# FuxiComputerVision/Nefii

Hardware: AMD Instinct MI355X
Metric: training rays/sec (Step-2 material opt) (higher is better)
Workload: dtype f16x3; 1 GPU; cfg3; parallelism=dp1, trace_tier=True, bracket_staged_eval=False, split_fp8=False, step_graph=False, cycle_batches=4, trace_prefetch=3, nonfinite_steps=0

## Files before the change

nefii_amd/csrc/nefii_mlp.hip:

```cpp
#include "mlp_tile.h"

using namespace nefii;

#define HIP_CHECK_LAUNCH()                       \
    do {                                         \
        hipError_t _e = hipGetLastError();       \
        if (_e != hipSuccess) return (int)_e;    \
    } while (0)

static inline int round32(int v) { return (v + 31) & ~31; }
static inline int pad_hidden(int v) { return v <= 32 ? round32(v) : (v + 63) & ~63; }
extern "C" int nefii_padded_width(int v) { return v < 0 ? NEFII_E_ARG : pad_hidden(v); }

extern "C" int nefii_abi_version(void) { return NEFII_ABI_VERSION; }

struct PackGeom {
    int n_out, k_in, kx, ke, n_pad, x_src0, x_len, e_src0, e_len;
    float scale;
    __device__ __forceinline__ int src_col(int kk) const {
        if (kk < kx) return kk < x_len ? x_src0 + kk : -1;
        const int e = kk - kx;
        return e < e_len ? e_src0 + e : -1;
    }
    __device__ __forceinline__ float at(const float *__restrict__ W, int n, int kk) const {
// ... 771 lines not shown
                        const int j = ft * QT + qt;
                        float4v hv;
#pragma unroll
                        for (int k = 0; k < 4; ++k) {
                            const float z = __builtin_fmaf(acc[j][k], inv_scale, bs[k]);
                            hv[k] = ACT == NEFII_ACT_ELU ? elu_fast(z) : act_fwd(z, ACT);
                        }
                        const int64_t row = base + 16 * qt + (lane & 15);
                        if (row < n) {
                            if (stash) *reinterpret_cast<float4v *>(stash + ((size_t)l * n + row) * stash_stride + f0) = hv;
                            if (pre_last) {
#pragma unroll
                                for (int k = 0; k < 4; ++k)
                                    if (f0 + k < L.n_out) hidden_out[(size_t)row * hid_stride + f0 + k] = hv[k];
                            }
                        }
                        const float4v hs = hv * A16_SCALE;
                        const half4 hi = __builtin_convertvector(hs, half4);
                        phi[j] = hi;
                        plo[j] = __builtin_convertvector(hs - __builtin_convertvector(hi, float4v), half4);
                        if (H16 && stash16 && row < n)
                            *reinterpret_cast<half4 *>(stash16 + ((size_t)l * n + row) * stash_stride + f0) = hi;
                    }
                }
            };
            if (m.act == NEFII_ACT_RELU)
                epilogue(std::integral_constant<int, NEFII_ACT_RELU>{});
            else if (m.act == NEFII_ACT_ELU)
                epilogue(std::integral_constant<int, NEFII_ACT_ELU>{});
            else
                epilogue(std::integral_constant<int, NEFII_ACT_SOFTPLUS100>{});
            __syncthreads();
            _Float16 *xh = lds.Xh + (EP - L.n_pad), *xl = lds.Xl + (EP - L.n_pad);
#pragma unroll
            for (int ft = 0; ft < 4; ++ft) {
                const int f0 = 64 * wave + 16 * ft + 4 * (lane >> 4);
#pragma unroll
                for (int qt = 0; qt < QT; ++qt) {
                    const int query = 16 * qt + (lane & 15);
                    *reinterpret_cast<half4 *>(xh + query * XP + f0) = phi[ft * QT + qt];
                    *reinterpret_cast<half4 *>(xl + query * XP + f0) = plo[ft * QT + qt];
                }
            }
            __syncthreads();
        }
        {
            const int r = lane & 31, h = lane >> 5;
            const nefii_layer &L = m.layer[NH];
            const half8 *wl = reinterpret_cast<const half8 *>(L.w_f16x3) + lane;
            const int ksw = (L.k_x >> 4) / NW;
            f32x16 acc2[RT];
#pragma unroll
            for (int rt = 0; rt < RT; ++rt)
#pragma unroll
                for (int i = 0; i < 16; ++i) acc2[rt][i] = 0.f;
            for (int u = 0; u < ksw; ++u) {
                const int s = wave * ksw + u;
                const half8 wh = wl[(size_t)s * 128], wlo = wl[(size_t)s * 128 + 64];
#pragma unroll
                for (int rt = 0; rt < RT; ++rt) {
                    const int rowc = 32 * rt + r < ROWS ? 32 * rt + r : ROWS - 1;
                    const half8 xh8 = *reinterpret_cast<const half8 *>(lds.Xh + rowc * XP + 8 * h + 16 * s);
                    const half8 xl8 = *reinterpret_cast<const half8 *>(lds.Xl + rowc * XP + 8 * h + 16 * s);
                    acc2[rt] = __builtin_amdgcn_mfma_f32_32x32x16_f16(wh, xh8, acc2[rt], 0, 0, 0);
                    acc2[rt] = __builtin_amdgcn_mfma_f32_32x32x16_f16(wlo, xh8, acc2[rt], 0, 0, 0);
                    acc2[rt] = __builtin_amdgcn_mfma_f32_32x32x16_f16(wh, xl8, acc2[rt], 0, 0, 0);
                }
            }
            __syncthreads();
            float *psum = reinterpret_cast<float *>(lds.Xl);
#pragma unroll
            for (int rt = 0; rt < RT; ++rt)
                if (32 * rt + r < ROWS) {
#pragma unroll
                    for (int i = 0; i < 4; ++i) psum[(wave * ROWS + 32 * rt + r) * 8 + i + 4 * h] = acc2[rt][i];
                }
            __syncthreads();
            for (int i = tid; i < ROWS * 8; i += 512) {
                const int p = i >> 3, c = i & 7;
                if (c < L.n_out && base + p < n) {
                    float sum = 0.f;
#pragma unroll
                    for (int w = 0; w < NW; ++w) sum += psum[(w * ROWS + p) * 8 + c];
                    const float z = sum * inv_scale + L.bias[c];
                    if (stash) stash[((size_t)NH * n + base + p) * stash_stride + c] = z;
                    if (H16 && z_last) z_last[(size_t)(base + p) * 8 + c] = z;
                    out[(size_t)(base + p) * out_stride + c] = head_fwd(z, m.head);
                }
            }
            __syncthreads();
            for (int i = tid; i < NW * ROWS * 8; i += 512) reinterpret_cast<uint32_t *>(lds.Xl)[i] = 0u;
            __syncthreads();
        }
    }
}

static int check_mlp16(const nefii_mlp *m, bool bwd) {
    int rc = check_mlp(m, false);
    if (rc) return rc;
    for (int l = 0; l < m->n_layers; ++l) {
        if (!m->layer[l].w_f16x3) return NEFII_E_ARG;
        if (bwd && l > 0 && !m->layer[l].w_bwd_f16x3) return NEFII_E_ARG;
        if ((m->layer[l].k_x | m->layer[l].k_e | m->layer[l].n_pad) & 15) return NEFII_E_SHAPE;
    }
    return 0;
}

static bool mlp_stream_enabled() {
    static const bool v = env_int("NEFII_MLP_STREAM", 1) != 0;
    return v;
}
static bool mlp_streams_both_ways(const nefii_mlp *m) {
    return m->w_stream && mlp_stream_enabled() && mstream_shape(m) && mstream_units_bwd(m) > 0;
}
static dim3 stream_grid(int64_t n) {
    const int64_t t = (n + 63) / 64;
    return dim3((int)(t < 256 ? t : 256));
}

template <bool H16>
static int launch_forward16q(const nefii_mlp *h_mlp, const float *in_a, const float *in_b, const float *in_c, const float *feat,
                             int64_t n, float *out, int out_stride, float *hidden_out, int hid_stride, void *stash,
                             int stash_stride, float *z_last, void *x0_16, void *stream) {
    const auto kernel = mstream_shape(h_mlp) == 64 ? mlp_forward16q_kernel<4, 64, H16> : mlp_forward16q_kernel<4, 96, H16>;
    hipLaunchKernelGGL(kernel, stream_grid(n), dim3(512), 0, (hipStream_t)stream, *h_mlp, in_a, in_b, in_c, feat, n, out,
                       out_stride, hidden_out, hid_stride, stash, stash_stride, z_last, (_Float16 *)x0_16, mstream_units(h_mlp));
    HIP_CHECK_LAUNCH();
    return 0;
}

extern "C" int nefii_mlp_forward_f16(const nefii_mlp *h_mlp, const float *in_a, const float *in_b, const float *in_c,
                                     const float *feat, int64_t n, float *out, int out_stride, float *hidden_out,
                                     int hid_stride, float *stash, int stash_stride, int single_pass, void *stream) {
    int rc = check_mlp16(h_mlp, false);
    if (rc) return rc;
    if (n <= 0) return 0;
    if (!out) return NEFII_E_ARG;
    const int64_t n_tiles = (n + TILE - 1) / TILE;
    if (!single_pass && h_mlp->w_stream && mlp_stream_enabled() && mstream_shape(h_mlp))
        return launch_forward16q<false>(h_mlp, in_a, in_b, in_c, feat, n, out, out_stride, hidden_out, hid_stride, stash,
                                        stash_stride, nullptr, nullptr, stream);
    if (single_pass)
        hipLaunchKernelGGL(mlp_forward16_kernel<true>, dim3(grid_for(n_tiles, 1)), dim3(WG), 0, (hipStream_t)stream, *h_mlp,
                           in_a, in_b, in_c, feat, n, out, out_stride, hidden_out, hid_stride, stash, stash_stride);
    else
        hipLaunchKernelGGL(mlp_forward16_kernel<false>, dim3(grid_for(n_tiles, 1)), dim3(WG), 0, (hipStream_t)stream, *h_mlp,
                           in_a, in_b, in_c, feat, n, out, out_stride, hidden_out, hid_stride, stash, stash_stride);
    HIP_CHECK_LAUNCH();
    return 0;
}

extern "C" int nefii_mlp_h16_supported(const nefii_mlp *h_mlp) {
    if (!h_mlp || check_mlp16(h_mlp, true)) return 0;
    return mlp_streams_both_ways(h_mlp);
}

extern "C" int nefii_mlp_x0_width(const nefii_mlp *h_mlp) {
    if (!nefii_mlp_h16_supported(h_mlp)) return 0;
    return h_mlp->layer[0].k_x + mstream_shape(h_mlp);
}

extern "C" int nefii_mlp_forward_f16h(const nefii_mlp *h_mlp, const float *in_a, const float *in_b, const float *in_c,
                                      const float *feat, int64_t n, float *out, int out_stride, float *hidden_out,
                                      int hid_stride, void *stash16, int stash_stride, float *z_last, void *x0_16,
                                      void *stream) {
    int rc = check_mlp16(h_mlp, false);
    if (rc) return rc;
    if (!nefii_mlp_h16_supported(h_mlp)) return NEFII_E_SHAPE;
    if (n <= 0) return 0;
    if (!out || !stash16 || !z_last || (stash_stride & 3)) return NEFII_E_ARG;
    return launch_forward16q<true>(h_mlp, in_a, in_b, in_c, feat, n, out, out_stride, hidden_out, hid_stride, stash16,
                                   stash_stride, z_last, x0_16, stream);
}

__global__ void grad_scale_kernel(const float *__restrict__ d, int64_t count, float *__restrict__ scale) {
    __shared__ float wmax[16];
    float mx = 0.f;
    for (int64_t i = threadIdx.x; i < count; i += blockDim.x) {
        const float v = fabsf(d[i]);
        mx = (v < 3.0e38f && v > mx) ? v : mx;
    }
#pragma unroll
    for (int o = 32; o > 0; o >>= 1) mx = fmaxf(mx, __shfl_xor(mx, o));
    if ((threadIdx.x & 63) == 0) wmax[threadIdx.x >> 6] = mx;
    __syncthreads();
    if (threadIdx.x == 0) {
        for (int w = 1; w < (int)(blockDim.x >> 6); ++w) mx = fmaxf(mx, wmax[w]);
        float s = 1.f;
        if (mx > 0.f) {
            int e;
            frexpf(mx, &e);
            e = 8 - e;
            e = e < -40 ? -40 : (e > 60 ? 60 : e);
            s = ldexpf(1.f, e);
        }
        scale[0] = s;
    }
}

__global__ void grad_scale_head_kernel(const float *__restrict__ d, int out_stride, const float *__restrict__ pre, int pre_stride,
                                       int64_t n, int n_out, int head, float *__restrict__ scale) {
    __shared__ float wmax[16];
    float mx = 0.f;
    const int64_t count = n * n_out;
    for (int64_t i = threadIdx.x; i < count; i += blockDim.x) {
        const int64_t p = i / n_out;
        const int c = (int)(i - p * n_out);
        const float dv = d[p * out_stride + c], z = pre[p * pre_stride + c];
        const float v = fabsf(dv);
        const float hv = fabsf(dv * head_bwd_from_out(head_fwd(z, head), z, head)) * 0.125f;
        mx = (v < 3.0e38f && v > mx) ? v : mx;
        mx = (hv < 3.0e38f && hv > mx) ? hv : mx;
    }
#pragma unroll
    for (int o = 32; o > 0; o >>= 1) mx = fmaxf(mx, __shfl_xor(mx, o));
    if ((threadIdx.x & 63) == 0) wmax[threadIdx.x >> 6] = mx;
    __syncthreads();
    if (threadIdx.x == 0) {
        for (int w = 1; w < (int)(blockDim.x >> 6); ++w) mx = fmaxf(mx, wmax[w]);
        float s = 1.f;
        if (mx > 0.f) {
            int e;
            frexpf(mx, &e);
            e = 8 - e;
            e = e < -40 ? -40 : (e > 60 ? 60 : e);
            s = ldexpf(1.f, e);
        }
        scale[0] = s;
    }
}

extern "C" int nefii_mlp_grad_scale_head(const float *d_out, int out_stride, const float *pre, int pre_stride, int64_t n,
                                         int n_out, int head, float *scale, void *stream) {
    if (!d_out || !pre || !scale || n < 0 || n_out < 1 || out_stride < n_out || pre_stride < n_out) return NEFII_E_ARG;
    if (head < NEFII_HEAD_NONE || head > NEFII_HEAD_RELU_INIT) return NEFII_E_ARG;
    hipLaunchKernelGGL(grad_scale_head_kernel, dim3(1), dim3(1024), 0, (hipStream_t)stream, d_out, out_stride, pre, pre_stride, n,
                       n_out, head, scale);
    HIP_CHECK_LAUNCH();
    return 0;
}

extern "C" int nefii_mlp_grad_scale(const float *d_out, int64_t count, float *scale, void *stream) {
    if (!d_out || !scale || count < 0) return NEFII_E_ARG;
    hipLaunchKernelGGL(grad_scale_kernel, dim3(1), dim3(1024), 0, (hipStream_t)stream, d_out, count, scale);
    HIP_CHECK_LAUNCH();
    return 0;
}

__global__ __launch_bounds__(256, 2) void mlp_backward16_kernel(nefii_mlp m, const float *__restrict__ d_out,
                                                                int out_stride, const float *__restrict__ stash,
                                                                int stash_stride, int64_t n, float *__restrict__ dz,
                                                                int dz_stride, const float *__restrict__ scale) {
    __shared__ _Float16 Xh[TILE * XS16];
    const int tid = threadIdx.x;
    const int Lm1 = m.n_layers - 1;
    const float S = scale[0];
    const float inv = 1.f / (W16_SCALE * S);
    const int64_t n_tiles = (n + TILE - 1) / TILE;
    for (int64_t tile = blockIdx.x; tile < n_tiles; tile += gridDim.x) {
        const int64_t base = tile * TILE;
        {
            const nefii_layer &L = m.layer[Lm1];
            for (int i = tid; i < TILE * L.n_pad; i += WG) {
                const int p = i / L.n_pad, c = i - p * L.n_pad;
                float v = 0.f;
                if (base + p < n && c < L.n_out) {
                    const float pre = stash[((size_t)Lm1 * n + base + p) * stash_stride + c];
                    const float y = head_fwd(pre, m.head);
                    v = d_out[(size_t)(base + p) * out_stride + c] * head_bwd_from_out(y, pre, m.head);
                }
                Xh[p * XS16 + c] = (_Float16)(v * S);
                if (base + p < n) dz[((size_t)Lm1 * n + base + p) * dz_stride + c] = v;
            }
        }
        __syncthreads();
        for (int l = Lm1; l >= 1; --l) {
            const nefii_layer &L = m.layer[l];
            f32x16 acc[4];
            const int wave = __builtin_amdgcn_readfirstlane(tid >> 6), lane = tid & 63;
            const int NTs = (L.k_x + L.k_e) >> 5, ntc = L.k_x >> 5;
            int ntw = (ntc - wave + 3) >> 2;
            if (ntw < 0) ntw = 0;
            zero_acc(acc);
            gemm_block16<true>(Xh, Xh, XS16, L.n_pad >> 4, reinterpret_cast<const half8 *>(L.w_bwd_f16x3), NTs, wave, lane,
                               ntw, acc);
            __syncthreads();
            NEFII_ACT_SWITCH(m.act, {
                NEFII_FOR_ACC(acc, ntw, {
                    const bool live = (base + row) < n;
                    float v = 0.f;
                    if (live) {
                        const float hprev = stash[((size_t)(l - 1) * n + base + row) * stash_stride + col];
                        v = val * inv * act_bwd_from_out(hprev, ACT);
                        dz[((size_t)(l - 1) * n + base + row) * dz_stride + col] = v;
                    }
                    Xh[row * XS16 + col] = (_Float16)(v * S);
                })
            })
            __syncthreads();
        }
    }
}

template <bool H16>
__global__ __launch_bounds__(512, 2) void mlp_backward16s_kernel(nefii_mlp m, const float *__restrict__ d_out, int out_stride,
                                                                const void *__restrict__ stash_v, int stash_stride,
                                                                const float *__restrict__ z_last, int64_t n,
                                                                void *__restrict__ dz_v, int dz_stride,
                                                                const float *__restrict__ scale, size_t stream_off, int G) {
    NEFII_CLAIM_SIMD_2();
    const float *const stash = static_cast<const float *>(stash_v);
    const _Float16 *const stash16 = static_cast<const _Float16 *>(stash_v);
    float *const dz = static_cast<float *>(dz_v);
    _Float16 *const dz16 = static_cast<_Float16 *>(dz_v);
    constexpr int QT = 4, FT = 4, ROWS = 64, XP = QGeo<4>::XP, NJ = FT * QT;
    __shared__ LdsS<4, ROWS> lds;
    const int tid = threadIdx.x;
    const int wave = __builtin_amdgcn_readfirstlane(tid >> 6), lane = tid & 63;
    const int Lm1 = m.n_layers - 1;
    const float S = scale[0];
    const float inv = 1.f / (W16_SCALE * S);
    const int64_t n_tiles = (n + ROWS - 1) / ROWS;
    {
        uint32_t *z = reinterpret_cast<uint32_t *>(&lds);
        for (int i = tid; i < (int)(sizeof(lds) / 4); i += 512) z[i] = 0u;
    }
    SStage<4> b[4];
    PCursor cur;
    cur.bytes = (unsigned)G * 4096;
    cur.base = reinterpret_cast<const half8 *>(m.w_stream) + stream_off + (size_t)wave * G * 256 + lane;
    cur.off = 0;
#pragma unroll
    for (int u = 0; u < 3; ++u) sload<4>(b[u], cur);
    const _Float16 *qh0 = lds.Xh + (lane & 15) * XP + 8 * (lane >> 4);
    __syncthreads();
    for (int64_t tile = blockIdx.x; tile < n_tiles; tile += gridDim.x) {
        const int64_t base = tile * ROWS;
        {
            const nefii_layer &L = m.layer[Lm1];
            const int kpad = mb_units(L) * 32;
            for (int i = tid; i < ROWS * kpad; i += 512) {
                const int p = i / kpad, c = i - p * kpad;
                float v = 0.f;
                if (base + p < n && c < L.n_pad) {
                    if (c < L.n_out) {
                        const float pre = H16 ? z_last[(size_t)(base + p) * 8 + c]
                                              : stash[((size_t)Lm1 * n + base + p) * stash_stride + c];
                        const float y = head_fwd(pre, m.head);
                        v = d_out[(size_t)(base + p) * out_stride + c] * head_bwd_from_out(y, pre, m.head);
                    }
                    if (H16) dz16[((size_t)Lm1 * n + base + p) * dz_stride + c] = (_Float16)(v * S);
                    else dz[((size_t)Lm1 * n + base + p) * dz_stride + c] = v;
                }
                lds.Xh[p * XP + c] = (_Float16)(v * S);
            }
        }
        __syncthreads();
        for (int l = Lm1; l >= 1; --l) {
            const nefii_layer &L = m.layer[l];
            const int units = mb_units(L);
            asm volatile("" ::"s"(units));
            __builtin_amdgcn_s_waitcnt(0x0070);
            __builtin_amdgcn_sched_barrier(0);
            f32x4 acc[NJ];
#pragma unroll
            for (int j = 0; j < NJ; ++j)
#pragma unroll
                for (int i = 0; i < 4; ++i) acc[j][i] = 0.f;
            SAct<QT> a[2];
            sload_a<QT, XP>(a[0], qh0, 0);
            sgemm<QT, FT, true>(units, b, a, cur, qh0, acc);
            half4 phi[NJ];
            const float *sp = stash + (size_t)(l - 1) * n * stash_stride;
            float *dp = dz + (size_t)(l - 1) * n * dz_stride;
            const _Float16 *sp16 = stash16 + (size_t)(l - 1) * n * stash_stride;
            _Float16 *dp16 = dz16 + (size_t)(l - 1) * n * dz_stride;
            auto epilogue = [&](auto actc) {
                constexpr int ACT = decltype(actc)::value;
#pragma unroll
                for (int ft = 0; ft < FT; ++ft) {
                    const int f0 = 64 * wave + 16 * ft + 4 * (lane >> 4);
#pragma unroll
                    for (int qt = 0; qt < QT; ++qt) {
                        const int j = ft * QT + qt;
                        const int64_t row = base + 16 * qt + (lane & 15);
                        float4v v = {0.f, 0.f, 0.f, 0.f};
                        if (row < n) {
                            float4v h;
                            if (H16)
                                h = __builtin_convertvector(*reinterpret_cast<const half4 *>(sp16 + (size_t)row * stash_stride + f0),
                                                            float4v) * (1.f / A16_SCALE);
                            else
                                h = *reinterpret_cast<const float4v *>(sp + (size_t)row * stash_stride + f0);
#pragma unroll
                            for (int k = 0; k < 4; ++k) v[k] = acc[j][k] * inv * act_bwd_from_out(h[k], ACT);
                            if (!H16) *reinterpret_cast<float4v *>(dp + (size_t)row * dz_stride + f0) = v;
                        }
                        phi[j] = __builtin_convertvector(v * S, half4);
                        if (H16 && row < n) *reinterpret_cast<half4 *>(dp16 + (size_t)row * dz_stride + f0) = phi[j];
                    }
                }
            };
            if (m.act == NEFII_ACT_RELU)
                epilogue(std::integral_constant<int, NEFII_ACT_RELU>{});
            else if (m.act == NEFII_ACT_ELU)
                epilogue(std::integral_constant<int, NEFII_ACT_ELU>{});
            else
                epilogue(std::integral_constant<int, NEFII_ACT_SOFTPLUS100>{});
            __syncthreads();
#pragma unroll
            for (int ft = 0; ft < FT; ++ft) {
                const int f0 = 64 * wave + 16 * ft + 4 * (lane >> 4);
#pragma unroll
                for (int qt = 0; qt < QT; ++qt)
                    *reinterpret_cast<half4 *>(lds.Xh + (16 * qt + (lane & 15)) * XP + f0) = phi[ft * QT + qt];
            }
            __syncthreads();
        }
    }
}

template <bool H16>
static int launch_backward16s(const nefii_mlp *h_mlp, const float *d_out, int out_stride, const void *stash, int stash_stride,
                              const float *z_last, int64_t n, void *dz, int dz_stride, const float *scale, void *stream) {
    hipLaunchKernelGGL(mlp_backward16s_kernel<H16>, stream_grid(n), dim3(512), 0, (hipStream_t)stream, *h_mlp, d_out, out_stride,
                       stash, stash_stride, z_last, n, dz, dz_stride, scale, (size_t)8 * mstream_units(h_mlp) * 256,
                       mstream_units_bwd(h_mlp));
    HIP_CHECK_LAUNCH();
    return 0;
}

extern "C" int nefii_mlp_backward_f16(const nefii_mlp *h_mlp, const float *d_out, int out_stride, const float *stash,
                                      int stash_stride, int64_t n, float *dz, int dz_stride, const float *scale,
                                      void *stream) {
    int rc = check_mlp16(h_mlp, true);
    if (rc) return rc;
    if (n <= 0) return 0;
    if (!d_out || !stash || !dz || !scale) return NEFII_E_ARG;
    if (mlp_streams_both_ways(h_mlp) && (stash_stride & 3) == 0 && (dz_stride & 3) == 0)
        return launch_backward16s<false>(h_mlp, d_out, out_stride, stash, stash_stride, nullptr, n, dz, dz_stride, scale, stream);
    const int64_t n_tiles = (n + TILE - 1) / TILE;
    hipLaunchKernelGGL(mlp_backward16_kernel, dim3(grid_for(n_tiles, 2)), dim3(WG), 0, (hipStream_t)stream, *h_mlp, d_out,
                       out_stride, stash, stash_stride, n, dz, dz_stride, scale);
    HIP_CHECK_LAUNCH();
    return 0;
}

extern "C" int nefii_mlp_backward_f16h(const nefii_mlp *h_mlp, const float *d_out, int out_stride, const void *stash16,
                                       int stash_stride, const float *z_last, int64_t n, void *dz16, int dz_stride,
                                       const float *scale, void *stream) {
    int rc = check_mlp16(h_mlp, true);
    if (rc) return rc;
    if (!nefii_mlp_h16_supported(h_mlp)) return NEFII_E_SHAPE;
    if (n <= 0) return 0;
    if (!d_out || !stash16 || !z_last || !dz16 || !scale || (stash_stride & 3) || (dz_stride & 3)) return NEFII_E_ARG;
    return launch_backward16s<true>(h_mlp, d_out, out_stride, stash16, stash_stride, z_last, n, dz16, dz_stride, scale, stream);
}

template <bool DZ16, bool X16>
__device__ __forceinline__ void wgrad16_body(const void *__restrict__ dz_v, int dz_stride, const void *__restrict__ x_v,
                                             int x_stride, int64_t P, int n_out, int k_in, float scale,
                                             const float *__restrict__ gscale, float *__restrict__ dW, float *__restrict__ db,
                                             int atomic, int bx, int by, int bz, int gz) {
    const float *const dz = static_cast<const float *>(dz_v), *const x = static_cast<const float *>(x_v);
    const _Float16 *const dz16 = static_cast<const _Float16 *>(dz_v), *const x16 = static_cast<const _Float16 *>(x_v);
    const int wave = threadIdx.x >> 6, lane = threadIdx.x & 63;
    const int i = lane & 31, h = lane >> 5;
    const int n0 = bx * 64 + (wave & 1) * 32;
    const int k0 = by * 256 + (wave >> 1) * 128;
    const int64_t chunk = ((P + gz - 1) / gz + 15) & ~(int64_t)15;
    const int64_t p_begin = (int64_t)bz * chunk;
    const int64_t p_end = p_begin + chunk < P ? p_begin + chunk : P;
    const float S = gscale[0];
    f32x16 acc[4];
    zero_acc(acc);
    const bool n_ok = (n0 + i) < n_out;
    bool k_ok[4];
#pragma unroll
    for (int t = 0; t < 4; ++t) k_ok[t] = (k0 + 32 * t + i) < k_in;
    float bsum = 0.f;
    if (n0 < n_out && k0 < k_in) {
        const int nc = n_ok ? n0 + i : n_out - 1;
        int kc[4];
#pragma unroll
        for (int t = 0; t < 4; ++t) kc[t] = k_ok[t] ? k0 + 32 * t + i : k_in - 1;
        const int64_t p_last = p_end - 1;
        constexpr int U = 2;
        for (int64_t pb = p_begin; pb < p_end; pb += 16 * U) {
            float a[U][8], b[U][4][8];
#pragma unroll
            for (int u = 0; u < U; ++u)
#pragma unroll
                for (int j = 0; j < 8; ++j) {
                    const int64_t p = pb + 16 * u + 8 * h + j;
                    const int64_t pc = p < p_last ? p : p_last;
                    a[u][j] = DZ16 ? (float)dz16[pc * dz_stride + nc] : dz[pc * dz_stride + nc];
#pragma unroll
                    for (int t = 0; t < 4; ++t) b[u][t][j] = X16 ? (float)x16[pc * x_stride + kc[t]] : x[pc * x_stride + kc[t]];
                }
#pragma unroll
            for (int u = 0; u < U; ++u) {
                half8 af;
#pragma unroll
                for (int j = 0; j < 8; ++j) {
                    const bool ok = (pb + 16 * u + 8 * h + j) < p_end && n_ok;
                    const float av = ok ? a[u][j] : 0.f;
                    bsum += av;
                    af[j] = DZ16 ? (_Float16)av : (_Float16)(av * S);
                }
#pragma unroll
                for (int t = 0; t < 4; ++t) {
                    half8 bf;
#pragma unroll
                    for (int j = 0; j < 8; ++j) bf[j] = (_Float16)(k_ok[t] ? b[u][t][j] : 0.f);
                    acc[t] = __builtin_amdgcn_mfma_f32_32x32x16_f16(af, bf, acc[t], 0, 0, 0);
                }
            }
        }
        const float os = scale / S * (X16 ? 1.f / A16_SCALE : 1.f);
#pragma unroll
        for (int t = 0; t < 4; ++t)
#pragma unroll
            for (int r = 0; r < 16; ++r) {
                const int nn = n0 + (r & 3) + 8 * (r >> 2) + 4 * h, k = k0 + 32 * t + i;
                if (nn < n_out && k < k_in) {
                    const float v = acc[t][r] * os;
                    if (atomic) atomicAdd(&dW[(size_t)nn * k_in + k], v);
                    else dW[(size_t)nn * k_in + k] = v;
                }
            }
    }
    if (db && by == 0 && (wave >> 1) == 0) {
        bsum += __shfl_xor(bsum, 32);
        if (DZ16) bsum /= S;
        if (h == 0 && n_ok) {
            if (atomic) atomicAdd(&db[n0 + i], bsum);
            else db[n0 + i] = bsum;
        }
    }
}

template <bool DZ16, bool X16>
__global__ __launch_bounds__(256) void mlp_wgrad16_kernel(const void *__restrict__ dz_v, int dz_stride,
                                                          const void *__restrict__ x_v, int x_stride, int64_t P, int n_out,
                                                          int k_in, float scale, const float *__restrict__ gscale,
                                                          float *__restrict__ dW, float *__restrict__ db, int atomic) {
    wgrad16_body<DZ16, X16>(dz_v, dz_stride, x_v, x_stride, P, n_out, k_in, scale, gscale, dW, db, atomic, blockIdx.x, blockIdx.y,
                            blockIdx.z, gridDim.z);
}

constexpr int WG2_ROWS = 32, WG2_STRIDE = 160, WG2_POINTS = 4096;
typedef short short4v __attribute__((ext_vector_type(4)));

__device__ __forceinline__ half8 wg2_fragment(const _Float16 *tile, int col0, int row0, int lane) {
    const int l16 = lane & 15, q = l16 >> 2, pp = l16 & 3;
    const _Float16 *a = tile + (row0 + 8 * (lane >> 5) + q) * WG2_STRIDE + col0 + 16 * ((lane >> 4) & 1) + 4 * pp;
    typedef short4v __attribute__((address_space(3))) * lds_ptr;
    const short4v lo = __builtin_amdgcn_ds_read_tr16_b64_v4i16((lds_ptr)(a));
    const short4v hi = __builtin_amdgcn_ds_read_tr16_b64_v4i16((lds_ptr)(a + 4 * WG2_STRIDE));
    const half4 l4 = __builtin_bit_cast(half4, lo), h4 = __builtin_bit_cast(half4, hi);
    return half8{l4[0], l4[1], l4[2], l4[3], h4[0], h4[1], h4[2], h4[3]};
}

template <bool XVEC, bool DZ16, bool X16>
__device__ __forceinline__ void wgrad16t_body(const void *__restrict__ dz_v, int dz_stride, const void *__restrict__ x_v,
                                              int x_stride, int64_t P, int n_out, int k_in, float scale,
                                              const float *__restrict__ gscale, float *__restrict__ dW, float *__restrict__ db,
                                              int splits, int tiles_n, int tiles_k, unsigned bid) {
    __shared__ __attribute__((aligned(16))) _Float16 A[2][WG2_ROWS * WG2_STRIDE], B[2][WG2_ROWS * WG2_STRIDE];
    const float *const dz = static_cast<const float *>(dz_v), *const x = static_cast<const float *>(x_v);
    const _Float16 *const dz16 = static_cast<const _Float16 *>(dz_v), *const x16 = static_cast<const _Float16 *>(x_v);
    const int nt = tiles_n * tiles_k;
    const int xcd = bid & 7, j = bid >> 3;
    const int tile = j % nt, slice = 8 * (j / nt) + xcd;
    if (slice >= splits) return;
    const int tn = tile % tiles_n, tk = tile / tiles_n;
    const int n0 = 128 * tn, k0 = 128 * tk;
    const int tid = threadIdx.x, wave = tid >> 6, lane = tid & 63;
    const int64_t chunk = ((P + splits - 1) / splits + WG2_ROWS - 1) / WG2_ROWS * WG2_ROWS;
    const int64_t p_begin = (int64_t)slice * chunk;
    const int64_t p_end = p_begin + chunk < P ? p_begin + chunk : P;
    if (p_begin >= p_end) return;
    const float S = gscale[0];
    const int c4 = tid & 31, r8 = tid >> 5;
    const int c8 = tid & 15, r16 = tid >> 4;
    const int na = n0 + (DZ16 ? 8 * c8 : 4 * c4), ka = k0 + (X16 ? 8 * c8 : 4 * c4);
    const bool n_in = na + (DZ16 ? 7 : 3) < n_out, k_in_ok = ka + (X16 ? 7 : 3) < k_in;
    float4v ra[4], rb[4];
    half8 ha[2], hb[2];
    float bsum[8] = {0.f, 0.f, 0.f, 0.f, 0.f, 0.f, 0.f, 0.f};
    const half8 hzero = {0, 0, 0, 0, 0, 0, 0, 0};
    auto fetch = [&](int64_t pb) {
        if (DZ16) {
#pragma unroll
            for (int u = 0; u < 2; ++u) {
                const int64_t pr = pb + r16 + 16 * u;
                const int64_t pc = pr < p_end ? pr : p_end - 1;
                half8 a = hzero;
                if (n_in) {
                    a = *reinterpret_cast<const half8 *>(dz16 + pc * dz_stride + na);
                } else {
#pragma unroll
                    for (int e = 0; e < 8; ++e) a[e] = dz16[pc * dz_stride + (na + e < n_out ? na + e : n_out - 1)];
#pragma unroll
                    for (int e = 0; e < 8; ++e) a[e] = na + e < n_out ? a[e] : (_Float16)0;
                }
                ha[u] = pr < p_end ? a : hzero;
            }
        } else {
#pragma unroll
            for (int u = 0; u < 4; ++u) {
                const int64_t pr = pb + r8 + 8 * u;
                const int64_t pc = pr < p_end ? pr : p_end - 1;
                float4v a = {0.f, 0.f, 0.f, 0.f};
                if (n_in) {
                    a = *reinterpret_cast<const float4v *>(dz + pc * dz_stride + na);
                } else {
#pragma unroll
                    for (int e = 0; e < 4; ++e) a[e] = dz[pc * dz_stride + (na + e < n_out ? na + e : n_out - 1)];
#pragma unroll
                    for (int e = 0; e < 4; ++e) a[e] = na + e < n_out ? a[e] : 0.f;
                }
                ra[u] = pr < p_end ? a : float4v{0.f, 0.f, 0.f, 0.f};
            }
        }
        if (X16) {
#pragma unroll
            for (int u = 0; u < 2; ++u) {
                const int64_t pr = pb + r16 + 16 * u;
                const int64_t pc = pr < p_end ? pr : p_end - 1;
                half8 b = hzero;
                if (XVEC && k_in_ok) {
                    b = *reinterpret_cast<const half8 *>(x16 + pc * x_stride + ka);
                } else {
#pragma unroll
                    for (int e = 0; e < 8; ++e) b[e] = x16[pc * x_stride + (ka + e < k_in ? ka + e : k_in - 1)];
#pragma unroll
                    for (int e = 0; e < 8; ++e) b[e] = ka + e < k_in ? b[e] : (_Float16)0;
                }
                hb[u] = pr < p_end ? b : hzero;
            }
        } else {
#pragma unroll
            for (int u = 0; u < 4; ++u) {
                const int64_t pr = pb + r8 + 8 * u;
                const int64_t pc = pr < p_end ? pr : p_end - 1;
                float4v b = {0.f, 0.f, 0.f, 0.f};
                if (XVEC && k_in_ok) {
                    b = *reinterpret_cast<const float4v *>(x + pc * x_stride + ka);
                } else {
#pragma unroll
                    for (int e = 0; e < 4; ++e) b[e] = x[pc * x_stride + (ka + e < k_in ? ka + e : k_in - 1)];
#pragma unroll
                    for (int e = 0; e < 4; ++e) b[e] = ka + e < k_in ? b[e] : 0.f;
                }
                rb[u] = pr < p_end ? b : float4v{0.f, 0.f, 0.f, 0.f};
            }
        }
    };
    auto stage = [&](int buf) {
        if (DZ16) {
#pragma unroll
            for (int u = 0; u < 2; ++u) {
#pragma unroll
                for (int e = 0; e < 8; ++e) bsum[e] += (float)ha[u][e];
                *reinterpret_cast<half8 *>(&A[buf][(r16 + 16 * u) * WG2_STRIDE + 8 * c8]) = ha[u];
            }
        } else {
#pragma unroll
            for (int u = 0; u < 4; ++u) {
#pragma unroll
                for (int e = 0; e < 4; ++e) bsum[e] += ra[u][e];
                *reinterpret_cast<half4 *>(&A[buf][(r8 + 8 * u) * WG2_STRIDE + 4 * c4]) = __builtin_convertvector(ra[u] * S, half4);
            }
        }
        if (X16) {
#pragma unroll
            for (int u = 0; u < 2; ++u) *reinterpret_cast<half8 *>(&B[buf][(r16 + 16 * u) * WG2_STRIDE + 8 * c8]) = hb[u];
        } else {
#pragma unroll
            for (int u = 0; u < 4; ++u)
                *reinterpret_cast<half4 *>(&B[buf][(r8 + 8 * u) * WG2_STRIDE + 4 * c4]) = __builtin_convertvector(rb[u], half4);
        }
    };
    f32x16 acc[4];
    zero_acc(acc);
    const int an = 64 * (wave & 1), bk = 64 * (wave >> 1);
    fetch(p_begin);
    stage(0);
    __syncthreads();
    int buf = 0;
    for (int64_t pb = p_begin; pb < p_end; pb += WG2_ROWS) {
        const bool more = pb + WG2_ROWS < p_end;
        if (more) fetch(pb + WG2_ROWS);
#pragma unroll
        for (int ks = 0; ks < 2; ++ks) {
            half8 af[2], bf[2];
#pragma unroll
            for (int t = 0; t < 2; ++t) {
                af[t] = wg2_fragment(A[buf], an + 32 * t, 16 * ks, lane);
                bf[t] = wg2_fragment(B[buf], bk + 32 * t, 16 * ks, lane);
            }
#pragma unroll
            for (int t = 0; t < 2; ++t)
#pragma unroll
                for (int v = 0; v < 2; ++v)
                    acc[2 * t + v] = __builtin_amdgcn_mfma_f32_32x32x16_f16(af[t], bf[v], acc[2 * t + v], 0, 0, 0);
        }
        if (more) stage(buf ^ 1);
        __syncthreads();
        buf ^= 1;
    }
    const float os = scale / S * (X16 ? 1.f / A16_SCALE : 1.f);
    const int i = lane & 31, h = lane >> 5;
#pragma unroll
    for (int t = 0; t < 2; ++t)
#pragma unroll
        for (int v = 0; v < 2; ++v)
#pragma unroll
            for (int r = 0; r < 16; ++r) {
                const int nn = n0 + an + 32 * t + (r & 3) + 8 * (r >> 2) + 4 * h, k = k0 + bk + 32 * v + i;
                if (nn < n_out && k < k_in) atomicAdd(&dW[(size_t)nn * k_in + k], acc[2 * t + v][r] * os);
            }
    if (db && tk == 0) {
        __syncthreads();
        float *red = reinterpret_cast<float *>(&A[0][0]);
        if (DZ16) {
#pragma unroll
// ... 425 lines not shown
```

Baseline: 1.908 million rays/s.

## Double-buffer LDS activation image and prefetch stash in streamed MLP backward

Adds an EPI variant of the streamed backward MLP kernel, on by default through an environment variable. It keeps two LDS activation images, so each layer's epilogue writes the next layer's input directly into the other buffer. This drops one __syncthreads per layer and the separate phi copy pass. It also issues the stash loads for the activation derivative before the GEMM in the f16 case, and with vector loads in the f32 case, to hide their global latency. The cost is double the LDS footprint, which may reduce occupancy, plus more registers for the prefetched values.

```diff
diff --git a/nefii_amd/csrc/nefii_mlp.hip b/nefii_amd/csrc/nefii_mlp.hip
--- a/nefii_amd/csrc/nefii_mlp.hip
+++ b/nefii_amd/csrc/nefii_mlp.hip
@@ -1097,7 +1097,7 @@
     }
 }
 
-template <bool H16>
+template <bool H16, bool EPI>
 __global__ __launch_bounds__(512, 2) void mlp_backward16s_kernel(nefii_mlp m, const float *__restrict__ d_out, int out_stride,
                                                                 const void *__restrict__ stash_v, int stash_stride,
                                                                 const float *__restrict__ z_last, int64_t n,
@@ -1109,7 +1109,11 @@
     float *const dz = static_cast<float *>(dz_v);
     _Float16 *const dz16 = static_cast<_Float16 *>(dz_v);
     constexpr int QT = 4, FT = 4, ROWS = 64, XP = QGeo<4>::XP, NJ = FT * QT;
-    __shared__ LdsS<4, ROWS> lds;
+    __shared__ std::conditional_t<EPI, LdsS2<4, ROWS>, LdsS<4, ROWS>> lds;
+    auto image = [&](int i) -> _Float16 * {
+        if constexpr (EPI) return lds.X[i & 1];
+        else return lds.Xh;
+    };
     const int tid = threadIdx.x;
     const int wave = __builtin_amdgcn_readfirstlane(tid >> 6), lane = tid & 63;
     const int Lm1 = m.n_layers - 1;
@@ -1127,12 +1131,14 @@
     cur.off = 0;
 #pragma unroll
     for (int u = 0; u < 3; ++u) sload<4>(b[u], cur);
-    const _Float16 *qh0 = lds.Xh + (lane & 15) * XP + 8 * (lane >> 4);
+    const int qoff = (lane & 15) * XP + 8 * (lane >> 4);
+    const _Float16 *qh0 = image(0) + qoff;
     __syncthreads();
     for (int64_t tile = blockIdx.x; tile < n_tiles; tile += gridDim.x) {
         const int64_t base = tile * ROWS;
         {
             const nefii_layer &L = m.layer[Lm1];
+            _Float16 *const xs = image(Lm1);
             const int kpad = mb_units(L) * 32;
             for (int i = tid; i < ROWS * kpad; i += 512) {
                 const int p = i / kpad, c = i - p * kpad;
@@ -1147,13 +1153,92 @@
                     if (H16) dz16[((size_t)Lm1 * n + base + p) * dz_stride + c] = (_Float16)(v * S);
                     else dz[((size_t)Lm1 * n + base + p) * dz_stride + c] = v;
                 }
-                lds.Xh[p * XP + c] = (_Float16)(v * S);
+                xs[p * XP + c] = (_Float16)(v * S);
             }
         }
         __syncthreads();
         for (int l = Lm1; l >= 1; --l) {
             const nefii_layer &L = m.layer[l];
             const int units = mb_units(L);
+            if constexpr (EPI) {
+                const _Float16 *ah = lds.X[l & 1] + qoff;
+                _Float16 *xw = lds.X[(l & 1) ^ 1];
+                asm volatile("" ::"s"(units), "v"(ah), "v"(xw));
+                __builtin_amdgcn_s_waitcnt(0x0070);
+                __builtin_amdgcn_sched_barrier(0);
+                const int c0 = 64 * wave + 4 * (lane >> 4);
+                int64_t rowc[QT];
+#pragma unroll
+                for (int qt = 0; qt < QT; ++qt) {
+                    const int64_t row = base + 16 * qt + (lane & 15);
+                    rowc[qt] = row < n ? row : n - 1;
+                }
+                half4 pre16[H16 ? NJ : 1];
+                if constexpr (H16) {
+                    const _Float16 *sp16 = stash16 + (size_t)(l - 1) * n * stash_stride + c0;
+#pragma unroll
+                    for (int qt = 0; qt < QT; ++qt)
+#pragma unroll
+                        for (int ft = 0; ft < FT; ++ft)
+                            pre16[ft * QT + qt] = *reinterpret_cast<const half4 *>(sp16 + (size_t)rowc[qt] * stash_stride + 16 * ft);
+                    __builtin_amdgcn_sched_barrier(0);
+                }
+                f32x4 acc[NJ];
+#pragma unroll
+                for (int j = 0; j < NJ; ++j)
+#pragma unroll
+                    for (int i = 0; i < 4; ++i) acc[j][i] = 0.f;
+                SAct<QT> a[2];
+                sload_a<QT, XP>(a[0], ah, 0);
+                sgemm<QT, FT, true>(units, b, a, cur, ah, acc);
+                float4v pre32[H16 ? 1 : NJ];
+                if constexpr (!H16) {
+                    const float *sp = stash + (size_t)(l - 1) * n * stash_stride + c0;
+#pragma unroll
+                    for (int qt = 0; qt < QT; ++qt)
+#pragma unroll
+                        for (int ft = 0; ft < FT; ++ft)
+                            pre32[ft * QT + qt] = *reinterpret_cast<const float4v *>(sp + (size_t)rowc[qt] * stash_stride + 16 * ft);
+                    __builtin_amdgcn_sched_barrier(0);
+                }
+                float *dp = dz + (size_t)(l - 1) * n * dz_stride + c0;
+                _Float16 *dp16 = dz16 + (size_t)(l - 1) * n * dz_stride + c0;
+                auto epilogue2 = [&](auto actc) {
+                    constexpr int ACT = decltype(actc)::value;
+#pragma unroll
+                    for (int ft = 0; ft < FT; ++ft) {
+#pragma unroll
+                        for (int qt = 0; qt < QT; ++qt) {
+                            const int j = ft * QT + qt;
+                            const int64_t row = base + 16 * qt + (lane & 15);
+                            const bool live = row < n;
+                            float4v h;
+                            if constexpr (H16) h = __builtin_convertvector(pre16[j], float4v) * (1.f / A16_SCALE);
+                            else h = pre32[j];
+                            float4v v;
+#pragma unroll
+                            for (int k = 0; k < 4; ++k) {
+                                const float g = acc[j][k] * inv * act_bwd_from_out(h[k], ACT);
+                                v[k] = live ? g : 0.f;
+                            }
+                            const half4 packed = __builtin_convertvector(v * S, half4);
+                            *reinterpret_cast<half4 *>(xw + (16 * qt + (lane & 15)) * XP + c0 + 16 * ft) = packed;
+                            if (live) {
+                                if constexpr (H16) *reinterpret_cast<half4 *>(dp16 + (size_t)row * dz_stride + 16 * ft) = packed;
+                                else *reinterpret_cast<float4v *>(dp + (size_t)row * dz_stride + 16 * ft) = v;
+                            }
+                        }
+                    }
+                };
+                if (m.act == NEFII_ACT_RELU)
+                    epilogue2(std::integral_constant<int, NEFII_ACT_RELU>{});
+                else if (m.act == NEFII_ACT_ELU)
+                    epilogue2(std::integral_constant<int, NEFII_ACT_ELU>{});
+                else
+                    epilogue2(std::integral_constant<int, NEFII_ACT_SOFTPLUS100>{});
+                __syncthreads();
+                continue;
+            }
             asm volatile("" ::"s"(units));
             __builtin_amdgcn_s_waitcnt(0x0070);
             __builtin_amdgcn_sched_barrier(0);
@@ -1208,7 +1293,7 @@
                 const int f0 = 64 * wave + 16 * ft + 4 * (lane >> 4);
 #pragma unroll
                 for (int qt = 0; qt < QT; ++qt)
-                    *reinterpret_cast<half4 *>(lds.Xh + (16 * qt + (lane & 15)) * XP + f0) = phi[ft * QT + qt];
+                    *reinterpret_cast<half4 *>(image(0) + (16 * qt + (lane & 15)) * XP + f0) = phi[ft * QT + qt];
             }
             __syncthreads();
         }
@@ -1218,7 +1303,8 @@
 template <bool H16>
 static int launch_backward16s(const nefii_mlp *h_mlp, const float *d_out, int out_stride, const void *stash, int stash_stride,
                               const float *z_last, int64_t n, void *dz, int dz_stride, const float *scale, void *stream) {
-    hipLaunchKernelGGL(mlp_backward16s_kernel<H16>, stream_grid(n), dim3(512), 0, (hipStream_t)stream, *h_mlp, d_out, out_stride,
+    const auto kernel = env_int("NEFII_HIT_EPILOGUE", 1) != 0 ? mlp_backward16s_kernel<H16, true> : mlp_backward16s_kernel<H16, false>;
+    hipLaunchKernelGGL(kernel, stream_grid(n), dim3(512), 0, (hipStream_t)stream, *h_mlp, d_out, out_stride,
                        stash, stash_stride, z_last, n, dz, dz_stride, scale, (size_t)8 * mstream_units(h_mlp) * 256,
                        mstream_units_bwd(h_mlp));
     HIP_CHECK_LAUNCH();
```

Result: no change. 1.914 million rays/s, median of 6 (+0.3%).
